# TuringLang/Bijectors.jl

Measured on NVIDIA B200. Metric: samples/sec: with_logabsdet_jacobian through 8-layer Planar flow, D=128, higher is better.
Workload: dtype f32

## Files before the change

### bijectors.jl_b200/csrc/b2b_planar_common.cuh

```cuda
#pragma once
#include <cstring>

#include "b2b_v1_pipeline.cuh"

namespace b2b {

constexpr int HP_MAX_L = 8;
constexpr int HP_MAX_D = 128;

template <int D, int L>
__device__ __forceinline__ void planar_derive_smem(const B2BChainParams& P, int nreal, float* params, int warp, int lane,
                                                   int nw) {
  for (int l = warp; l < L; l += nw) {
    float* w_out = params + l * D;
    float* u_out = params + L * D + l * D;
    if (l >= nreal) {
      for (int i = lane; i < D; i += 32) w_out[i] = u_out[i] = 0.f;
      if (lane == 0) params[2 * L * D + l] = params[2 * L * D + L + l] = 0.f;
      continue;
    }
    const b2b_layer_desc& d = P.layers[l];
    float s = 0.f, q = 0.f;
    for (int i = lane; i < D; i += 32) {
      const float w = d.p0[i], u = d.p1[i];
      s = fmaf(w, u, s);
      q = fmaf(w, w, q);
    }
    s = warp_sum(s);
    q = warp_sum(q);
    const float k = (softplus(-s) - 1.0f) / q;
    for (int i = lane; i < D; i += 32) {
      const float w = d.p0[i];
      w_out[i] = w;
      u_out[i] = fmaf(k, w, d.p1[i]);
    }
    if (lane == 0) {
      params[2 * L * D + l] = softplus(s) - 1.0f;
      params[2 * L * D + L + l] = d.p2[0];
    }
  }
}

static __global__ void __launch_bounds__(HP_MAX_L * 32)
    planar_prep_kernel(const __grid_constant__ B2BChainParams P, int L, int Lp, float* __restrict__ out) {
  const int lane = threadIdx.x & 31, l = threadIdx.x >> 5, D = P.D;
  if (l >= Lp) return;
  auto put = [&](int idx, float v) { out[idx] = v; };
  const int wo = l * D, uo = Lp * D + l * D;
  if (l >= L) {
    for (int i = lane; i < D; i += 32) {
      put(wo + i, 0.f);
      put(uo + i, 0.f);
    }
    if (lane == 0) {
      put(2 * Lp * D + l, 0.f);
      put(2 * Lp * D + Lp + l, 0.f);
    }
    return;
  }
  const b2b_layer_desc& d = P.layers[l];
  float s = 0.f, q = 0.f;
  for (int i = lane; i < D; i += 32) {
    const float w = d.p0[i], u = d.p1[i];
    s = fmaf(w, u, s);
    q = fmaf(w, w, q);
  }
  s = warp_sum(s);
  q = warp_sum(q);
  const float k = (softplus(-s) - 1.0f) / q;
  for (int i = lane; i < D; i += 32) {
    const float w = d.p0[i];
    put(wo + i, w);
    put(uo + i, fmaf(k, w, d.p1[i]));
  }
  if (lane == 0) {
    put(2 * Lp * D + l, softplus(s) - 1.0f);
    put(2 * Lp * D + Lp + l, d.p2[0]);
  }
}

struct HPShape {
  int nw, mode;
};

static HPShape hp_shape(int D, int L) {
  HPShape s;
  s.nw = D == 128 ? 8 : (D == 64 ? 12 : 16);
  s.mode = (2 * D * L * 4 > 4096) ? 2 : 0;
  return s;
}

}
```

### bijectors.jl_b200/csrc/b2b_planar_const.cu

```cuda
#include "b2b_planar_common.cuh"

namespace b2b {

template <int D, int L>
struct PlanarHP {
  float v[2 * L * D + 2 * L];
};

template <int D, int L>
struct ArgSrc {
  static constexpr bool kDerive = false;
  const PlanarHP<D, L>& H;
  int invmask;
  __device__ __forceinline__ float w(int l, int i) const { return H.v[l * D + i]; }
  __device__ __forceinline__ float uh(int l, int i) const { return H.v[L * D + l * D + i]; }
  __device__ __forceinline__ float c(int l) const { return H.v[2 * L * D + l]; }
  __device__ __forceinline__ float b(int l) const { return H.v[2 * L * D + L + l]; }
  __device__ __forceinline__ bool inv(int l) const { return (invmask >> l) & 1; }
  __device__ __forceinline__ float raw(int i) const { return H.v[i]; }
};

template <int D, int L>
struct DevSrc {
  static constexpr bool kDerive = true;
  int invmask, nreal;
  __device__ __forceinline__ bool inv(int l) const { return (invmask >> l) & 1; }
};

template <int D, int L, int MODE, int DIR, bool MVN, class Src>
struct PlanarConstProg {
  using State = V1NoState;
  const Src src;
  const B2BChainParams& P;
  static constexpr bool DERIVE = Src::kDerive;
  static constexpr int NPK = 2 * L * D + 2 * L;
  static constexpr bool STAGED = MODE != 0 || DERIVE;
  static constexpr int MVN_OFF = STAGED ? ((NPK + 3) & ~3) : 0;
  static constexpr bool TAB = DERIVE && DIR != 0;
  static constexpr int TAB_OFF = MVN_OFF + (MVN ? 2 * D + 4 : 0);
  static constexpr int SMEM_FLOATS = TAB_OFF + (TAB ? L * PT_FLOATS : 0);
  __device__ __forceinline__ void stage(float* params, int warp, int lane, int nw) const {
    if constexpr (DERIVE) {
      if (MVN && warp == nw - 1) stage_layer(P.layers[src.nreal], params + MVN_OFF, D, D, lane);
      planar_derive_smem<D, L>(P, src.nreal, params, warp, lane, nw);
      if constexpr (TAB) {
        __syncthreads();
        for (int idx = warp * 32 + lane; idx < L * PT_N; idx += nw * 32) {
          const int l = idx / PT_N;
          if (DIR == 1 || src.inv(l)) planar_table_piece(params[2 * L * D + l], idx - l * PT_N, params + TAB_OFF + l * PT_FLOATS);
        }
      }
    } else if constexpr (STAGED) {
      for (int i = warp * 32 + lane; i < NPK; i += nw * 32) params[i] = src.raw(i);
    }
  }

  template <bool WS, bool US, bool SS>
  __device__ __forceinline__ void layers(float2 (&x)[1][D / 2], const float* params, float (&lj)[1]) const {
#pragma unroll
    for (int l = 0; l < L; ++l) {
      const float4* w4 = reinterpret_cast<const float4*>(params + l * D);
      const float4* u4 = reinterpret_cast<const float4*>(params + L * D + l * D);
      float2 acc[4];
#pragma unroll
      for (int i = 0; i < 4; ++i) acc[i] = make_float2(0.f, 0.f);
#pragma unroll
      for (int i = 0; i < D / 4; ++i) {
        float4 w;
        if constexpr (WS) w = w4[i];
        else w = make_float4(src.w(l, 4 * i), src.w(l, 4 * i + 1), src.w(l, 4 * i + 2), src.w(l, 4 * i + 3));
        acc[(i & 1) * 2 + 0] = __ffma2_rn(make_float2(w.x, w.y), x[0][2 * i], acc[(i & 1) * 2 + 0]);
        acc[(i & 1) * 2 + 1] = __ffma2_rn(make_float2(w.z, w.w), x[0][2 * i + 1], acc[(i & 1) * 2 + 1]);
      }
      const float2 s = __fadd2_rn(__fadd2_rn(acc[0], acc[1]), __fadd2_rn(acc[2], acc[3]));
      const float wz = s.x + s.y;
      float cc_, bb;
      if constexpr (SS) {
        cc_ = params[2 * L * D + l];
        bb = params[2 * L * D + L + l];
      } else {
        cc_ = src.c(l);
        bb = src.b(l);
      }
      float t, s2;
      if (DIR == 0 || (DIR == 2 && !src.inv(l))) {
        tanh_sech2(wz + bb, t, s2);
        lj[0] += log1pf(cc_ * s2);
      } else {
        if constexpr (TAB) find_alpha_tab(wz, cc_, bb, params + TAB_OFF + l * PT_FLOATS, t, s2);
        else find_alpha_ts(wz, cc_, bb, t, s2);
        lj[0] -= log1pf(cc_ * s2);
        t = -t;
      }
      const float2 t2 = make_float2(t, t);
#pragma unroll
      for (int i = 0; i < D / 4; ++i) {
        float4 u;
        if constexpr (US) u = u4[i];
        else u = make_float4(src.uh(l, 4 * i), src.uh(l, 4 * i + 1), src.uh(l, 4 * i + 2), src.uh(l, 4 * i + 3));
        x[0][2 * i] = __ffma2_rn(make_float2(u.x, u.y), t2, x[0][2 * i]);
        x[0][2 * i + 1] = __ffma2_rn(make_float2(u.z, u.w), t2, x[0][2 * i + 1]);
      }
    }
  }

  __device__ __forceinline__ void apply(float2 (&x)[1][D / 2], const ColCtx<D, 1>& ctx, const float* params,
                                        float (&lj)[1]) const {
    if constexpr (DERIVE) layers<true, true, true>(x, params, lj);
    else layers<MODE == 2, MODE == 1, false>(x, params, lj);
    if (MVN) mvnormal_apply<D, 1, 1>(x, ctx, params + MVN_OFF, lj);
  }
};

template <int D, int L, int NW, int MODE, int DIR>
__global__ void __launch_bounds__(NW * 32, 1)
    planar_arg_kernel(const __grid_constant__ B2BChainParams P, const __grid_constant__ V1Extra E,
                      const __grid_constant__ CUtensorMap map_x, const __grid_constant__ CUtensorMap map_y,
                      const __grid_constant__ PlanarHP<D, L> H, const int invmask) {
  const PlanarConstProg<D, L, MODE, DIR, false, ArgSrc<D, L>> prog{{H, invmask}, P};
  v1_run<D, 1, 1, NW>(P, E, map_x, map_y, prog);
}

template <int D, int L, int NW, int DIR, bool MVN>
__global__ void __launch_bounds__(NW * 32, 1)
    planar_dev_kernel(const __grid_constant__ B2BChainParams P, const __grid_constant__ V1Extra E,
                      const __grid_constant__ CUtensorMap map_x, const __grid_constant__ CUtensorMap map_y,
                      const int invmask, const int nreal) {
  const PlanarConstProg<D, L, 0, DIR, MVN, DevSrc<D, L>> prog{{invmask, nreal}, P};
  v1_run<D, 1, 1, NW>(P, E, map_x, map_y, prog);
}

template <int D, int L, int NW, int MODE, int DIR>
static int launch_arg(const B2BChainParams& q, const V1Geom& g, const CUtensorMap& mx, const CUtensorMap& my,
                      const float* packed, int invmask, cudaStream_t stream) {
  static PlanarHP<D, L> H;
  static std::mutex mu;
  std::lock_guard<std::mutex> lock(mu);
  memcpy(H.v, packed, sizeof(H.v));
  auto kernel = planar_arg_kernel<D, L, NW, MODE, DIR>;
  cudaError_t e = cudaFuncSetAttribute(kernel, cudaFuncAttributeMaxDynamicSharedMemorySize, (int)g.smem);
  if (e != cudaSuccess) return (int)e;
  kernel<<<g.grid, NW * 32, g.smem, stream>>>(q, g.extra, mx, my, H, invmask);
  return (int)cudaGetLastError();
}

template <int D, int L, int NW, int DIR, bool MVN = false>
static int launch_dev(const B2BChainParams& q, const V1Geom& g, const CUtensorMap& mx, const CUtensorMap& my,
                      int nreal, int invmask, cudaStream_t stream) {
  auto kernel = planar_dev_kernel<D, L, NW, DIR, MVN>;
  cudaError_t e = cudaFuncSetAttribute(kernel, cudaFuncAttributeMaxDynamicSharedMemorySize, (int)g.smem);
  if (e != cudaSuccess) return (int)e;
  kernel<<<g.grid, NW * 32, g.smem, stream>>>(q, g.extra, mx, my, invmask, nreal);
  return (int)cudaGetLastError();
}

template <int D, int NW, int LL, int MM>
static int dispatch_arg_dir(const B2BChainParams& q, const V1Geom& g, const CUtensorMap& mx, const CUtensorMap& my,
                            const float* packed, int invmask, cudaStream_t stream) {
  const int all = (1 << LL) - 1;
  const int dir = (invmask & all) == 0 ? 0 : ((invmask & all) == all ? 1 : 2);
  if (dir == 0) return launch_arg<D, LL, NW, MM, 0>(q, g, mx, my, packed, invmask, stream);
  if (dir == 1) return launch_arg<D, LL, NW, MM, 1>(q, g, mx, my, packed, invmask, stream);
  return launch_arg<D, LL, NW, MM, 2>(q, g, mx, my, packed, invmask, stream);
}

template <int D, int NW>
static int dispatch_arg(int L, int mode, const B2BChainParams& q, const V1Geom& g, const CUtensorMap& mx,
                        const CUtensorMap& my, const float* packed, int invmask, cudaStream_t stream) {
  if (L == 1 && mode == 0) return dispatch_arg_dir<D, NW, 1, 0>(q, g, mx, my, packed, invmask, stream);
  if (L == 2 && mode == 0) return dispatch_arg_dir<D, NW, 2, 0>(q, g, mx, my, packed, invmask, stream);
  if (L == 4 && mode == 0) return dispatch_arg_dir<D, NW, 4, 0>(q, g, mx, my, packed, invmask, stream);
  if constexpr (2 * D * 8 * 4 > 4096) {
    if (L == 8 && mode == 2) return dispatch_arg_dir<D, NW, 8, 2>(q, g, mx, my, packed, invmask, stream);
  } else {
    if (L == 8 && mode == 0) return dispatch_arg_dir<D, NW, 8, 0>(q, g, mx, my, packed, invmask, stream);
  }
  return B2B_EUNSUPPORTED;
}

template <int D, int NW, int LL>
static int dispatch_dev_dir(const B2BChainParams& q, const V1Geom& g, const CUtensorMap& mx, const CUtensorMap& my,
                            int nreal, int invmask, bool mvn, cudaStream_t stream) {
  const int all = (1 << LL) - 1;
  const int dir = (invmask & all) == 0 ? 0 : ((invmask & all) == all ? 1 : 2);
  if (mvn) {
    if (dir == 1) return launch_dev<D, LL, NW, 1, true>(q, g, mx, my, nreal, invmask, stream);
    return B2B_EUNSUPPORTED;
  }
  if (dir == 0) return launch_dev<D, LL, NW, 0>(q, g, mx, my, nreal, invmask, stream);
  if (dir == 1) return launch_dev<D, LL, NW, 1>(q, g, mx, my, nreal, invmask, stream);
  return launch_dev<D, LL, NW, 2>(q, g, mx, my, nreal, invmask, stream);
}

template <int D, int NW>
static int dispatch_dev(int L, const B2BChainParams& q, const V1Geom& g, const CUtensorMap& mx, const CUtensorMap& my,
                        int nreal, int invmask, bool mvn, cudaStream_t stream) {
  switch (L) {
    case 1: return dispatch_dev_dir<D, NW, 1>(q, g, mx, my, nreal, invmask, mvn, stream);
    case 2: return dispatch_dev_dir<D, NW, 2>(q, g, mx, my, nreal, invmask, mvn, stream);
    case 3: return dispatch_dev_dir<D, NW, 3>(q, g, mx, my, nreal, invmask, mvn, stream);
    case 4: return dispatch_dev_dir<D, NW, 4>(q, g, mx, my, nreal, invmask, mvn, stream);
    case 5: return dispatch_dev_dir<D, NW, 5>(q, g, mx, my, nreal, invmask, mvn, stream);
    case 6: return dispatch_dev_dir<D, NW, 6>(q, g, mx, my, nreal, invmask, mvn, stream);
    case 7: return dispatch_dev_dir<D, NW, 7>(q, g, mx, my, nreal, invmask, mvn, stream);
    case 8: return dispatch_dev_dir<D, NW, 8>(q, g, mx, my, nreal, invmask, mvn, stream);
    default: return B2B_EUNSUPPORTED;
  }
}

static int launch_planar_unrolled(const B2BChainParams& p, int L, const float* packed, int nreal, int invmask, bool mvn,
                                  cudaStream_t stream) {
  B2BChainParams q = p;
  q.scratch_off = -1;
  if (!(q.D == 32 || q.D == 64 || q.D == 128)) return B2B_EUNSUPPORTED;
  if (v1_check_io(q) != 0) return B2B_EUNSUPPORTED;
  const HPShape sh = hp_shape(q.D, L);
  V1Geom g;
  const bool staged = sh.mode != 0 || !packed;
  const size_t pf = (staged ? (size_t)((2 * L * q.D + 2 * L + 3) & ~3) : 0) + (mvn ? 2 * q.D + 4 : 0) +
                    ((!packed && invmask != 0) ? (size_t)L * PT_FLOATS : 0);
  const int rc = v1_geometry(q.D, q.N, sh.nw, 32, pf, g);
  if (rc != 0) return rc;
  CUtensorMap mx, my;
  if (!make_maps(q, g.cols, &mx, &my, &g.extra.tma3d)) return B2B_EUNSUPPORTED;
  if (packed) {
    if (q.D == 128) return dispatch_arg<128, 8>(L, sh.mode, q, g, mx, my, packed, invmask, stream);
    if (q.D == 64) return dispatch_arg<64, 12>(L, sh.mode, q, g, mx, my, packed, invmask, stream);
    return dispatch_arg<32, 16>(L, sh.mode, q, g, mx, my, packed, invmask, stream);
  }
  if (q.D == 128) return dispatch_dev<128, 8>(L, q, g, mx, my, nreal, invmask, mvn, stream);
  if (q.D == 64) return dispatch_dev<64, 12>(L, q, g, mx, my, nreal, invmask, mvn, stream);
  return dispatch_dev<32, 16>(L, q, g, mx, my, nreal, invmask, mvn, stream);
}

}

int b2b_planar_const_grid_size(const B2BChainParams& p) {
  using namespace b2b;
  if (!(p.D == 32 || p.D == 64 || p.D == 128)) return 0;
  V1Geom g;
  const HPShape sh = hp_shape(p.D, 8);
  if (v1_geometry(p.D, p.N, sh.nw, 32, 0, g) != 0) return 0;
  return g.grid;
}

int b2b_launch_planar_hostparams(const B2BChainParams& p, int L, const float* packed, int invmask,
                                 cudaStream_t stream) {
  return b2b::launch_planar_unrolled(p, L, packed, L, invmask, false, stream);
}

int b2b_planar_const_layers(const B2BChainParams& p) {
  using namespace b2b;
  if (!(p.D == 32 || p.D == 64 || p.D == 128) || p.L < 1) return 0;
  const bool mvn = p.layers[p.L - 1].kind == B2B_MVNORMAL_DIAG;
  const int n = p.L - (mvn ? 1 : 0);
  if (n < 1 || n > HP_MAX_L) return 0;
  for (int l = 0; l < n; ++l) {
    if (p.layers[l].kind != B2B_PLANAR) return 0;
    if (mvn && !p.layers[l].inverse) return 0;
  }
  if (v1_check_io(p) != 0) return 0;
  return n;
}

int b2b_launch_planar_chain_const(const B2BChainParams& p, cudaStream_t stream) {
  using namespace b2b;
  const int n = b2b_planar_const_layers(p);
  if (n == 0) return B2B_EUNSUPPORTED;
  int invmask = 0;
  for (int l = 0; l < n; ++l)
    if (p.layers[l].inverse) invmask |= 1 << l;
  return launch_planar_unrolled(p, n, nullptr, n, invmask, p.L > n, stream);
}
```

### bijectors.jl_b200/csrc/b2b_v1_pipeline.cuh

```cuda
#pragma once
#include <cuda.h>
#include <cuda_runtime.h>

#include <cstdlib>
#include <mutex>

#include "b2b_device.cuh"

namespace b2b {

__device__ __forceinline__ uint32_t smem_u32(const void* p) {
  return static_cast<uint32_t>(__cvta_generic_to_shared(p));
}
__device__ __forceinline__ void mbar_init(uint32_t bar, uint32_t count) {
  asm volatile("mbarrier.init.shared::cta.b64 [%0], %1;" ::"r"(bar), "r"(count));
}
__device__ __forceinline__ void mbar_expect_tx(uint32_t bar, uint32_t bytes) {
  asm volatile("mbarrier.arrive.expect_tx.shared::cta.b64 _, [%0], %1;" ::"r"(bar), "r"(bytes) : "memory");
}
__device__ __forceinline__ void mbar_wait(uint32_t bar, uint32_t parity) {
  asm volatile(
      "{\n"
      ".reg .pred P1;\n"
      "B2B_WAIT:\n"
      "mbarrier.try_wait.parity.shared::cta.b64 P1, [%0], %1;\n"
      "@P1 bra B2B_DONE;\n"
      "bra B2B_WAIT;\n"
      "B2B_DONE:\n"
      "}\n" ::"r"(bar),
      "r"(parity)
      : "memory");
}
__device__ __forceinline__ void tma_load_2d(uint32_t dst, const CUtensorMap* map, int c0, int c1, uint32_t bar) {
  asm volatile(
      "cp.async.bulk.tensor.2d.shared::cluster.global.mbarrier::complete_tx::bytes [%0], [%1, {%2, %3}], [%4];" ::"r"(dst),
      "l"(reinterpret_cast<uint64_t>(map)), "r"(c0), "r"(c1), "r"(bar)
      : "memory");
}
__device__ __forceinline__ void tma_store_2d(const CUtensorMap* map, int c0, int c1, uint32_t src) {
  asm volatile("cp.async.bulk.tensor.2d.global.shared::cta.bulk_group [%0, {%1, %2}], [%3];" ::"l"(
                   reinterpret_cast<uint64_t>(map)),
               "r"(c0), "r"(c1), "r"(src)
               : "memory");
}
__device__ __forceinline__ void tma_load_3d(uint32_t dst, const CUtensorMap* map, int c0, int c1, int c2, uint32_t bar) {
  asm volatile(
      "cp.async.bulk.tensor.3d.shared::cluster.global.mbarrier::complete_tx::bytes [%0], [%1, {%2, %3, %4}], [%5];" ::"r"(dst),
      "l"(reinterpret_cast<uint64_t>(map)), "r"(c0), "r"(c1), "r"(c2), "r"(bar)
      : "memory");
}
__device__ __forceinline__ void tma_store_3d(const CUtensorMap* map, int c0, int c1, int c2, uint32_t src) {
  asm volatile("cp.async.bulk.tensor.3d.global.shared::cta.bulk_group [%0, {%1, %2, %3}], [%4];" ::"l"(
                   reinterpret_cast<uint64_t>(map)),
               "r"(c0), "r"(c1), "r"(c2), "r"(src)
               : "memory");
}
__device__ __forceinline__ void mbar_arrive(uint32_t bar) {
  asm volatile("mbarrier.arrive.shared::cta.b64 _, [%0];" ::"r"(bar) : "memory");
}
__device__ __forceinline__ void bulk_load_1d(uint32_t dst, const void* src, uint32_t bytes, uint32_t bar) {
  asm volatile("cp.async.bulk.shared::cluster.global.mbarrier::complete_tx::bytes [%0], [%1], %2, [%3];" ::"r"(dst),
               "l"(reinterpret_cast<uint64_t>(src)), "r"(bytes), "r"(bar)
               : "memory");
}
__device__ __forceinline__ void tma_commit() { asm volatile("cp.async.bulk.commit_group;" ::: "memory"); }
__device__ __forceinline__ void tma_wait_read0() { asm volatile("cp.async.bulk.wait_group.read 0;" ::: "memory"); }
__device__ __forceinline__ void tma_wait_all0() { asm volatile("cp.async.bulk.wait_group 0;" ::: "memory"); }
__device__ __forceinline__ void fence_proxy_async() { asm volatile("fence.proxy.async.shared::cta;" ::: "memory"); }
__device__ __forceinline__ void fence_mbar_init() { asm volatile("fence.mbarrier_init.release.cluster;" ::: "memory"); }
__device__ __forceinline__ void flag_store_release(int* p, int v) {
  asm volatile("st.release.cta.shared::cta.s32 [%0], %1;" ::"r"(smem_u32(p)), "r"(v) : "memory");
}
__device__ __forceinline__ int flag_load_acquire(const int* p) {
  int v;
  asm volatile("ld.acquire.cta.shared::cta.s32 %0, [%1];" : "=r"(v) : "r"(smem_u32(p)) : "memory");
  return v;
}

struct V1Extra {
  int n_in;
  int param_off;
  int bar_off;
  int nwarps;
  int tma3d;
  long long tiles;
};

template <int D, int TPC>
struct ColCtx {
  static constexpr int EPT = D / TPC;
  static constexpr int NQT = EPT / 32;
  int h, rot;
  __device__ __forceinline__ int prm(int ql, int r) const { return (h * NQT + ql) * 8 + (r ^ rot); }
  __device__ __forceinline__ int row(int ql, int r, int e) const { return prm(ql, r) * 4 + e; }
};

template <int TPC>
__device__ __forceinline__ float part_sum(float v) {
#pragma unroll
  for (int o = 1; o < TPC; o <<= 1) v += __shfl_xor_sync(0xffffffffu, v, o);
  return v;
}

#define B2B_FOR_SLOTS                        \
  _Pragma("unroll") for (int ql = 0; ql < C::NQT; ++ql) _Pragma("unroll") for (int r = 0; r < 8; ++r)
#define B2B_FOR_COLS _Pragma("unroll") for (int cc = 0; cc < CPT; ++cc)

template <int D, int TPC, int CPT>
__device__ __forceinline__ void radial_apply(float2 (&x)[CPT][D / TPC / 2], const ColCtx<D, TPC>& c, const float* sp,
                                             bool inverse, float (&lj)[CPT]) {
  using C = ColCtx<D, TPC>;
  const float4* z4 = reinterpret_cast<const float4*>(sp);
  const float alpha = sp[D], bhat = sp[D + 1], apb = sp[D + 2];
  const float2 m1 = make_float2(-1.f, -1.f);
  float2 acc[CPT][4];
  B2B_FOR_COLS {
#pragma unroll
    for (int i = 0; i < 4; ++i) acc[cc][i] = make_float2(0.f, 0.f);
  }
  B2B_FOR_SLOTS {
    const float4 z0 = z4[c.prm(ql, r)];
    const int i = (ql * 8 + r) * 2;
    B2B_FOR_COLS {
      const float2 d0 = __ffma2_rn(make_float2(z0.x, z0.y), m1, x[cc][i]);
      const float2 d1 = __ffma2_rn(make_float2(z0.z, z0.w), m1, x[cc][i + 1]);
      acc[cc][(r & 1) * 2 + 0] = __ffma2_rn(d0, d0, acc[cc][(r & 1) * 2 + 0]);
      acc[cc][(r & 1) * 2 + 1] = __ffma2_rn(d1, d1, acc[cc][(r & 1) * 2 + 1]);
    }
  }
  float2 g2[CPT];
  B2B_FOR_COLS {
    const float2 s = __fadd2_rn(__fadd2_rn(acc[cc][0], acc[cc][1]), __fadd2_rn(acc[cc][2], acc[cc][3]));
    const float nrm = sqrtf(part_sum<TPC>(s.x + s.y));
    float r_ = nrm;
    if (inverse) {
      const float a = apb - nrm;
      const float sq = sqrtf(fmaf(a, a, 4.0f * alpha * nrm));
      r_ = a > 0.f ? (2.0f * alpha * nrm) / (sq + a) : 0.5f * (sq - a);
    }
    const float hh = 1.0f / (alpha + r_);
    const float bh = bhat * hh;
    const float ljf = (float)(D - 1) * log1pf(bh) + log1pf(bh * alpha * hh);
    float g;
    if (!inverse) {
      g = bh;
      lj[cc] += ljf;
    } else {
      g = -bhat / (apb + r_);
      lj[cc] -= ljf;
    }
    g2[cc] = make_float2(g, g);
  }
  B2B_FOR_SLOTS {
    const float4 z0 = z4[c.prm(ql, r)];
    const int i = (ql * 8 + r) * 2;
    B2B_FOR_COLS {
      const float2 d0 = __ffma2_rn(make_float2(z0.x, z0.y), m1, x[cc][i]);
      const float2 d1 = __ffma2_rn(make_float2(z0.z, z0.w), m1, x[cc][i + 1]);
      x[cc][i] = __ffma2_rn(g2[cc], d0, x[cc][i]);
      x[cc][i + 1] = __ffma2_rn(g2[cc], d1, x[cc][i + 1]);
    }
  }
}

template <int D, int TPC, int CPT>
__device__ __forceinline__ void mvnormal_apply(const float2 (&x)[CPT][D / TPC / 2], const ColCtx<D, TPC>& c,
                                               const float* sp, float (&lj)[CPT]) {
  using C = ColCtx<D, TPC>;
  const float4* mu4 = reinterpret_cast<const float4*>(sp);
  const float4* is4 = reinterpret_cast<const float4*>(sp + D);
  const float2 m1 = make_float2(-1.f, -1.f);
  float2 acc[CPT][2];
  B2B_FOR_COLS acc[cc][0] = acc[cc][1] = make_float2(0.f, 0.f);
  B2B_FOR_SLOTS {
    const float4 mu = mu4[c.prm(ql, r)], is = is4[c.prm(ql, r)];
    const int i = (ql * 8 + r) * 2;
    B2B_FOR_COLS {
      const float2 z0 = __fmul2_rn(__ffma2_rn(make_float2(mu.x, mu.y), m1, x[cc][i]), make_float2(is.x, is.y));
      const float2 z1 = __fmul2_rn(__ffma2_rn(make_float2(mu.z, mu.w), m1, x[cc][i + 1]), make_float2(is.z, is.w));
      acc[cc][0] = __ffma2_rn(z0, z0, acc[cc][0]);
      acc[cc][1] = __ffma2_rn(z1, z1, acc[cc][1]);
    }
  }
  B2B_FOR_COLS {
    const float2 s = __fadd2_rn(acc[cc][0], acc[cc][1]);
    lj[cc] += sp[2 * D] - 0.5f * part_sum<TPC>(s.x + s.y);
  }
}

struct V1Gen {
  unsigned long long seed, offset;
  long long col0;
  const float* mu;
  const float* sigma;
};

__device__ __forceinline__ void philox4x32_10(uint32_t c0, uint32_t c1, uint32_t c2, uint32_t c3, uint32_t k0, uint32_t k1,
                                              uint32_t (&out)[4]) {
#pragma unroll
  for (int r = 0; r < 10; ++r) {
    const uint32_t hi0 = __umulhi(0xD2511F53u, c0), lo0 = 0xD2511F53u * c0;
    const uint32_t hi1 = __umulhi(0xCD9E8D57u, c2), lo1 = 0xCD9E8D57u * c2;
    c0 = hi1 ^ c1 ^ k0;
    c1 = lo1;
    c2 = hi0 ^ c3 ^ k1;
    c3 = lo0;
    k0 += 0x9E3779B9u;
    k1 += 0xBB67AE85u;
  }
  out[0] = c0;
  out[1] = c1;
  out[2] = c2;
  out[3] = c3;
}

__device__ __forceinline__ void box_muller(uint32_t a, uint32_t b, float& z0, float& z1) {
  const float u1 = fmaf(__uint2float_rn(a), 2.3283064365386963e-10f, 1.1641532182693481e-10f);
  const float u2 = fmaf(__uint2float_rn(b), 2.3283064365386963e-10f, 1.1641532182693481e-10f);
  const float r = sqrtf(-1.3862943611198906f * __log2f(u1));
  const float ang = 6.283185307179586f * u2 - 3.141592653589793f;
  z0 = -r * __cosf(ang);
  z1 = -r * __sinf(ang);
}

__device__ __forceinline__ float4 philox_normal4(const V1Gen& g, long long n, int k) {
  uint32_t o[4];
  philox4x32_10((uint32_t)n, (uint32_t)((unsigned long long)n >> 32), (uint32_t)k, (uint32_t)g.offset, (uint32_t)g.seed,
                (uint32_t)(g.seed >> 32), o);
  float4 z;
  box_muller(o[0], o[1], z.x, z.y);
  box_muller(o[2], o[3], z.z, z.w);
  return z;
}

struct V1NoState {};

template <int D, int TPC, int CPT, int NW, class Prog, int NIN = 1, bool GEN = false>
__device__ __forceinline__ void v1_run(const B2BChainParams& P, const V1Extra& E, const CUtensorMap& map_x,
                                       const CUtensorMap& map_y, const Prog& prog,
                                       const CUtensorMap* map_x2 = nullptr, const V1Gen* gen = nullptr) {
  using C = ColCtx<D, TPC>;
  constexpr int NQ = D / 32;
  constexpr int LPC = 32 / TPC;
  constexpr int COLS = LPC * CPT;
  constexpr int BOX_BYTES = COLS * 128;
  constexpr int TILE_BYTES = NQ * BOX_BYTES;
  constexpr int SLOT_BYTES = NIN * TILE_BYTES;
  extern __shared__ unsigned char smem_dyn[];
  unsigned char* smem_raw = smem_dyn + ((1024u - (smem_u32(smem_dyn) & 1023u)) & 1023u);
  unsigned char* in_base = smem_raw;
  unsigned char* out_base = smem_raw + (size_t)E.n_in * SLOT_BYTES;
  float* params = reinterpret_cast<float*>(smem_raw + E.param_off);
  uint64_t* bars = reinterpret_cast<uint64_t*>(smem_raw + E.bar_off);
  int* armed = reinterpret_cast<int*>(bars + 8);

  const int lane = threadIdx.x & 31, warp = __shfl_sync(0xffffffffu, (int)(threadIdx.x >> 5), 0);
  auto load_tile = [&](uint32_t dst, int col0, uint32_t bar) {
    if (E.tma3d) {
      tma_load_3d(dst, &map_x, 0, col0, 0, bar);
      if (NIN == 2) tma_load_3d(dst + TILE_BYTES, map_x2, 0, col0, 0, bar);
    } else {
#pragma unroll
      for (int q = 0; q < NQ; ++q) tma_load_2d(dst + q * BOX_BYTES, &map_x, q * 32, col0, bar);
      if (NIN == 2) {
#pragma unroll
        for (int q = 0; q < NQ; ++q) tma_load_2d(dst + TILE_BYTES + q * BOX_BYTES, map_x2, q * 32, col0, bar);
      }
    }
  };
  const long long my_tiles = (E.tiles - blockIdx.x + gridDim.x - 1) / gridDim.x;
  if (threadIdx.x == 0 && !GEN) {
    for (int i = 0; i < E.n_in; ++i) mbar_init(smem_u32(&bars[i]), 1);
    fence_mbar_init();
    for (int j = 0; j < E.n_in && j < my_tiles; ++j) {
      const uint32_t bar = smem_u32(&bars[j]);
      mbar_expect_tx(bar, SLOT_BYTES);
      const long long tile = blockIdx.x + (long long)j * gridDim.x;
      load_tile(smem_u32(in_base + (size_t)j * SLOT_BYTES), (int)(tile * COLS), bar);
      flag_store_release(&armed[j], j);
    }
  }
  prog.stage(params, warp, lane, NW);
  __syncthreads();

  C ctx;
  const int t = lane / TPC;
  ctx.h = lane % TPC;
  ctx.rot = ctx.h * (8 / TPC);
  unsigned char* my_out = out_base + (size_t)warp * TILE_BYTES;
  const int sw = (((t & 7) ^ ctx.rot) & 7) * 16;
  const int line = t * 128 + ctx.h * C::NQT * BOX_BYTES;
  double dsum = 0.0;
  bool store_pending = false;

  for (long long j = warp; j < my_tiles; j += NW) {
    const int buf = (int)(j % E.n_in);
    const uint32_t parity = (uint32_t)((j / E.n_in) & 1);
    const long long tile = blockIdx.x + j * gridDim.x;
    const long long col = tile * COLS + t;
    if constexpr (!GEN) {
      while (flag_load_acquire(&armed[buf]) != (int)j) __nanosleep(20);
      mbar_wait(smem_u32(&bars[buf]), parity);
    }

    float2 x[CPT][C::EPT / 2];
    auto load_fragment = [&](const unsigned char* src) {
      B2B_FOR_COLS {
        B2B_FOR_SLOTS {
          const float4 v =
              *reinterpret_cast<const float4*>(src + cc * (LPC * 128) + ql * BOX_BYTES + ((r * 16) ^ sw));
          x[cc][(ql * 8 + r) * 2] = make_float2(v.x, v.y);
          x[cc][(ql * 8 + r) * 2 + 1] = make_float2(v.z, v.w);
        }
      }
    };
    if constexpr (GEN) {
      B2B_FOR_COLS {
        const long long n = gen->col0 + col + cc * LPC;
        B2B_FOR_SLOTS {
          const int row0 = ctx.row(ql, r, 0);
          float4 z = philox_normal4(*gen, n, row0 >> 2);
          if (gen->sigma) {
            const float4 sg = __ldg(reinterpret_cast<const float4*>(gen->sigma + row0));
            z = make_float4(z.x * sg.x, z.y * sg.y, z.z * sg.z, z.w * sg.w);
          }
          if (gen->mu) {
            const float4 m = __ldg(reinterpret_cast<const float4*>(gen->mu + row0));
            z = make_float4(z.x + m.x, z.y + m.y, z.z + m.z, z.w + m.w);
          }
          x[cc][(ql * 8 + r) * 2] = make_float2(z.x, z.y);
          x[cc][(ql * 8 + r) * 2 + 1] = make_float2(z.z, z.w);
        }
      }
    } else {
      load_fragment(in_base + (size_t)buf * SLOT_BYTES + line);
    }
    typename Prog::State st;
    if constexpr (NIN == 2) {
      prog.phase1(x, ctx, params, st);
      load_fragment(in_base + (size_t)buf * SLOT_BYTES + TILE_BYTES + line);
    }
    if constexpr (!GEN) fence_proxy_async();
    __syncwarp();
    if (!GEN && lane == 0 && j + E.n_in < my_tiles) {
      const uint32_t bar = smem_u32(&bars[buf]);
      mbar_expect_tx(bar, SLOT_BYTES);
      const long long nt = blockIdx.x + (j + E.n_in) * gridDim.x;
      load_tile(smem_u32(in_base + (size_t)buf * SLOT_BYTES), (int)(nt * COLS), bar);
      flag_store_release(&armed[buf], (int)(j + E.n_in));
    }

    float lj[CPT];
    B2B_FOR_COLS {
      const long long cl = col + cc * LPC;
      lj[cc] = (P.accumulate && P.logjac && cl < P.N) ? P.logjac[cl] : 0.0f;
    }
    if constexpr (NIN == 2) prog.apply(x, ctx, params, lj, st, col);
    else prog.apply(x, ctx, params, lj);

    if (P.y) {
      if (store_pending) {
        if (lane == 0) tma_wait_read0();
        __syncwarp();
      }
      unsigned char* dst = my_out + line;
      B2B_FOR_COLS {
        B2B_FOR_SLOTS {
          const float2 a = x[cc][(ql * 8 + r) * 2], b = x[cc][(ql * 8 + r) * 2 + 1];
          *reinterpret_cast<float4*>(dst + cc * (LPC * 128) + ql * BOX_BYTES + ((r * 16) ^ sw)) =
              make_float4(a.x, a.y, b.x, b.y);
        }
      }
      fence_proxy_async();
      __syncwarp();
      if (lane == 0) {
        if (E.tma3d) {
          tma_store_3d(&map_y, 0, (int)(tile * COLS), 0, smem_u32(my_out));
        } else {
#pragma unroll
          for (int q = 0; q < NQ; ++q)
            tma_store_2d(&map_y, q * 32, (int)(tile * COLS), smem_u32(my_out + q * BOX_BYTES));
        }
        tma_commit();
      }
      store_pending = true;
    }
    if (ctx.h == 0) {
      B2B_FOR_COLS {
        const long long cl = col + cc * LPC;
        if (cl < P.N) {
          if (P.logjac && !(P.accumulate & 2)) P.logjac[cl] = lj[cc];
          dsum += (double)lj[cc];
        }
      }
    }
  }
  if (lane == 0 && store_pending) tma_wait_all0();

  if (P.partials) {
    __shared__ double red[32];
#pragma unroll
    for (int o = 16; o > 0; o >>= 1) dsum += __shfl_xor_sync(0xffffffffu, dsum, o);
    if (lane == 0) red[warp] = dsum;
    __syncthreads();
    if (threadIdx.x == 0) {
      double tt = 0.0;
      for (int w = 0; w < NW; ++w) tt += red[w];
      P.partials[blockIdx.x] = tt;
    }
  }
}

typedef CUresult (*encode_tiled_fn)(CUtensorMap*, CUtensorMapDataType, cuuint32_t, void*, const cuuint64_t*,
                                    const cuuint64_t*, const cuuint32_t*, const cuuint32_t*, CUtensorMapInterleave,
                                    CUtensorMapSwizzle, CUtensorMapL2promotion, CUtensorMapFloatOOBfill);

static inline encode_tiled_fn get_encode() {
  static encode_tiled_fn fn = nullptr;
  static std::once_flag once;
  std::call_once(once, [] {
    void* p = nullptr;
    cudaDriverEntryPointQueryResult q;
    if (cudaGetDriverEntryPoint("cuTensorMapEncodeTiled", &p, cudaEnableDefault, &q) == cudaSuccess &&
        q == cudaDriverEntryPointSuccess)
      fn = reinterpret_cast<encode_tiled_fn>(p);
  });
  return fn;
}

static inline bool make_map(CUtensorMap* m, const float* base, int D, long long N, long long ld, int cols, bool three_d) {
  encode_tiled_fn enc = get_encode();
  if (!enc) return false;
  const cuuint32_t estr[3] = {1, 1, 1};
  if (three_d) {
    const cuuint64_t dims[3] = {32, (cuuint64_t)N, (cuuint64_t)(D / 32)};
    const cuuint64_t strides[2] = {(cuuint64_t)ld * sizeof(float), 128};
    const cuuint32_t box[3] = {32, (cuuint32_t)cols, (cuuint32_t)(D / 32)};
    return enc(m, CU_TENSOR_MAP_DATA_TYPE_FLOAT32, 3, const_cast<float*>(base), dims, strides, box, estr,
               CU_TENSOR_MAP_INTERLEAVE_NONE, CU_TENSOR_MAP_SWIZZLE_128B, CU_TENSOR_MAP_L2_PROMOTION_L2_128B,
               CU_TENSOR_MAP_FLOAT_OOB_FILL_NONE) == CUDA_SUCCESS;
  }
  const cuuint64_t dims[2] = {(cuuint64_t)D, (cuuint64_t)N};
  const cuuint64_t strides[1] = {(cuuint64_t)ld * sizeof(float)};
  const cuuint32_t box[2] = {32, (cuuint32_t)cols};
  return enc(m, CU_TENSOR_MAP_DATA_TYPE_FLOAT32, 2, const_cast<float*>(base), dims, strides, box, estr,
             CU_TENSOR_MAP_INTERLEAVE_NONE, CU_TENSOR_MAP_SWIZZLE_128B, CU_TENSOR_MAP_L2_PROMOTION_L2_128B,
             CU_TENSOR_MAP_FLOAT_OOB_FILL_NONE) == CUDA_SUCCESS;
}

static inline bool make_maps(const B2BChainParams& q, int cols, CUtensorMap* mx, CUtensorMap* my, int* tma3d) {
  static const int force2d = getenv("B2B_V1_TMA") && atoi(getenv("B2B_V1_TMA")) == 2;
  for (int three_d = force2d ? 0 : 1; three_d >= 0; --three_d) {
    if (three_d && q.D == 32) continue;
    bool ok = make_map(mx, q.x, q.D, q.N, q.ldx, cols, three_d != 0);
    if (ok && q.y) ok = make_map(my, q.y, q.D, q.N, q.ldy, cols, three_d != 0);
    if (ok) {
      if (!q.y) *my = *mx;
      *tma3d = three_d;
      return true;
    }
  }
  return false;
}

struct V1Geom {
  int nw, grid, cols;
  size_t smem;
  V1Extra extra;
};

static inline int v1_check_io(const B2BChainParams& p) {
  if (p.N >= (1ll << 31) - 64) return B2B_EUNSUPPORTED;
  if ((p.ldx % 4) || (reinterpret_cast<uintptr_t>(p.x) & 15)) return B2B_EUNSUPPORTED;
  if (p.y && ((p.ldy % 4) || (reinterpret_cast<uintptr_t>(p.y) & 15))) return B2B_EUNSUPPORTED;
  return 0;
}

static inline int v1_geometry(int D, long long N, int nw, int cols, size_t param_floats, V1Geom& g,
                              int in_tiles = 1) {
  const int tile_bytes = D * 4 * cols;
  const size_t param_bytes = param_floats * sizeof(float);
  const size_t budget = 225 * 1024;
  const size_t fixed = (size_t)nw * tile_bytes + ((param_bytes + 15) & ~(size_t)15) + 16 * sizeof(uint64_t) + 1024;
  const size_t slot_bytes = (size_t)in_tiles * tile_bytes;
  if (fixed + 2 * slot_bytes > budget) return B2B_EUNSUPPORTED;
  int n_in = (int)((budget - fixed) / slot_bytes);
  if (n_in > 8) n_in = 8;
  g.nw = nw;
  g.cols = cols;
  g.extra.n_in = n_in;
  g.extra.nwarps = nw;
  g.extra.tma3d = 0;
  g.extra.param_off = n_in * (int)slot_bytes + nw * tile_bytes;
  g.extra.bar_off = g.extra.param_off + (int)((param_bytes + 15) & ~(size_t)15);
  g.extra.tiles = (N + cols - 1) / cols;
  g.smem = (size_t)g.extra.bar_off + 16 * sizeof(uint64_t) + 1024;
  int dev = 0, sms = 0;
  cudaGetDevice(&dev);
  cudaDeviceGetAttribute(&sms, cudaDevAttrMultiProcessorCount, dev);
  long long grid = sms;
  const long long want = (g.extra.tiles + nw - 1) / nw;
  if (grid > want) grid = want;
  if (grid < 1) grid = 1;
  g.grid = (int)grid;
  return 0;
}

}
```

Measured before the change: 5.543 billion.

## Add forward planar tile program with coupling matrix and in-place TMA output

For all-forward planar chains, all L projections w_l·x are computed up front from the input. Later layers' pre-activations are then recovered through a precomputed L×L coupling matrix of w_l·û_k dot products, so the serial dependency on the evolving state is removed. Each tile's columns are split across TPC lanes with shuffle reductions, and the output is written back into the input slot in place. That frees the per-warp output buffer and allows up to 16 pipeline stages. The cost is extra parameter derivation per block, a changed barrier layout, and more register pressure from the L×CPT accumulators.

Result: no change. 5.496 billion, median of 6 (-0.8%).

```diff
diff --git a/bijectors.jl_b200/csrc/b2b_planar_common.cuh b/bijectors.jl_b200/csrc/b2b_planar_common.cuh
--- a/bijectors.jl_b200/csrc/b2b_planar_common.cuh
+++ b/bijectors.jl_b200/csrc/b2b_planar_common.cuh
@@ -38,6 +38,18 @@
       params[2 * L * D + l] = softplus(s) - 1.0f;
       params[2 * L * D + L + l] = d.p2[0];
     }
+  }
+}
+
+template <int D, int L>
+__device__ __forceinline__ void planar_derive_coupling(const float* params, float* m, int warp, int lane, int nw) {
+  for (int idx = warp; idx < L * L; idx += nw) {
+    const int l = idx / L, k = idx - l * L;
+    if (k >= l) continue;
+    float s = 0.f;
+    for (int i = lane; i < D; i += 32) s = fmaf(params[l * D + i], params[L * D + k * D + i], s);
+    s = warp_sum(s);
+    if (lane == 0) m[idx] = s;
   }
 }
 
diff --git a/bijectors.jl_b200/csrc/b2b_planar_const.cu b/bijectors.jl_b200/csrc/b2b_planar_const.cu
--- a/bijectors.jl_b200/csrc/b2b_planar_const.cu
+++ b/bijectors.jl_b200/csrc/b2b_planar_const.cu
@@ -112,6 +112,124 @@
   }
 };
 
+template <int D, int L>
+struct PlanarFwdProg {
+  using State = V1NoState;
+  static constexpr bool kTileIO = true;
+  static constexpr int TPC = D / 32, CPT = 4, OWN = CPT / TPC;
+  static constexpr int M_OFF = (2 * L * D + 2 * L + 3) & ~3;
+  static constexpr int SMEM_FLOATS = M_OFF + L * L;
+  const B2BChainParams& P;
+
+  __device__ __forceinline__ void stage(float* params, int warp, int lane, int nw) const {
+    planar_derive_smem<D, L>(P, L, params, warp, lane, nw);
+    __syncthreads();
+    planar_derive_coupling<D, L>(params, params + M_OFF, warp, lane, nw);
+  }
+
+  __device__ __forceinline__ void tile(const unsigned char* src, unsigned char* dst, const ColCtx<D, TPC>& ctx, int sw,
+                                       const float* params, float (&lj)[OWN]) const {
+    using C = ColCtx<D, TPC>;
+    const float4* w4 = reinterpret_cast<const float4*>(params);
+    const float4* u4 = reinterpret_cast<const float4*>(params + L * D);
+    float2 acc[L][CPT];
+#pragma unroll
+    for (int l = 0; l < L; ++l) {
+      B2B_FOR_COLS acc[l][cc] = make_float2(0.f, 0.f);
+    }
+    B2B_FOR_SLOTS {
+      float4 v[CPT];
+      B2B_FOR_COLS v[cc] = *reinterpret_cast<const float4*>(src + v1_chunk<D, TPC, CPT>(cc, ql, r, sw));
+#pragma unroll
+      for (int l = 0; l < L; ++l) {
+        const float4 w = w4[l * (D / 4) + ctx.prm(ql, r)];
+        B2B_FOR_COLS {
+          acc[l][cc] = __ffma2_rn(make_float2(w.x, w.y), make_float2(v[cc].x, v[cc].y), acc[l][cc]);
+          acc[l][cc] = __ffma2_rn(make_float2(w.z, w.w), make_float2(v[cc].z, v[cc].w), acc[l][cc]);
+        }
+      }
+    }
+    float a[L][CPT];
+#pragma unroll
+    for (int l = 0; l < L; ++l) {
+      B2B_FOR_COLS a[l][cc] = acc[l][cc].x + acc[l][cc].y;
+    }
+#pragma unroll
+    for (int o = TPC / 2, n = CPT / 2; o >= 1; o >>= 1, n >>= 1) {
+      const bool hi = ctx.h & o;
+#pragma unroll
+      for (int k = 0; k < n; ++k) {
+#pragma unroll
+        for (int l = 0; l < L; ++l) {
+          const float send = hi ? a[l][k] : a[l][k + n], keep = hi ? a[l][k + n] : a[l][k];
+          a[l][k] = keep + __shfl_xor_sync(0xffffffffu, send, o);
+        }
+      }
+    }
+    const float* M = params + M_OFF;
+    float t[L][CPT];
+#pragma unroll
+    for (int k = 0; k < OWN; ++k) {
+#pragma unroll
+      for (int l = 0; l < L; ++l) {
+        float al = a[l][k];
+#pragma unroll
+        for (int m = 0; m < l; ++m) al = fmaf(M[l * L + m], t[m][k], al);
+        float s2;
+        tanh_sech2(al + params[2 * L * D + L + l], t[l][k], s2);
+        lj[k] += log1pf(params[2 * L * D + l] * s2);
+      }
+    }
+    if (!dst) return;
+#pragma unroll
+    for (int o = 1, n = OWN; o < TPC; o <<= 1, n <<= 1) {
+      const bool hi = ctx.h & o;
+#pragma unroll
+      for (int k = 0; k < n; ++k) {
+#pragma unroll
+        for (int l = 0; l < L; ++l) {
+          const float mine = t[l][k], other = __shfl_xor_sync(0xffffffffu, mine, o);
+          t[l][k] = hi ? other : mine;
+          t[l][k + n] = hi ? mine : other;
+        }
+      }
+    }
+    float2 t2[L][CPT];
+#pragma unroll
+    for (int l = 0; l < L; ++l) {
+      B2B_FOR_COLS t2[l][cc] = make_float2(t[l][cc], t[l][cc]);
+    }
+    constexpr int NS = C::NQT * 8;
+    float4 v[CPT];
+    B2B_FOR_COLS v[cc] = *reinterpret_cast<const float4*>(src + v1_chunk<D, TPC, CPT>(cc, 0, 0, sw));
+#pragma unroll
+    for (int s = 0; s < NS; ++s) {
+      const int ql = s / 8, r = s % 8;
+      float2 z[CPT][2];
+      B2B_FOR_COLS {
+        z[cc][0] = make_float2(v[cc].x, v[cc].y);
+        z[cc][1] = make_float2(v[cc].z, v[cc].w);
+      }
+      if (s + 1 < NS) {
+        B2B_FOR_COLS v[cc] = *reinterpret_cast<const float4*>(src + v1_chunk<D, TPC, CPT>(cc, (s + 1) / 8, (s + 1) % 8, sw));
+      }
+#pragma unroll
+      for (int l = 0; l < L; ++l) {
+        const float4 u = u4[l * (D / 4) + ctx.prm(ql, r)];
+        B2B_FOR_COLS {
+          z[cc][0] = __ffma2_rn(make_float2(u.x, u.y), t2[l][cc], z[cc][0]);
+          z[cc][1] = __ffma2_rn(make_float2(u.z, u.w), t2[l][cc], z[cc][1]);
+        }
+      }
+      B2B_FOR_COLS *reinterpret_cast<float4*>(dst + v1_chunk<D, TPC, CPT>(cc, ql, r, sw)) =
+          make_float4(z[cc][0].x, z[cc][0].y, z[cc][1].x, z[cc][1].y);
+    }
+  }
+};
+
+constexpr int FWD_NW = 8;
+static inline int fwd_cols(int D) { return 4096 / D; }
+
 template <int D, int L, int NW, int MODE, int DIR>
 __global__ void __launch_bounds__(NW * 32, 1)
     planar_arg_kernel(const __grid_constant__ B2BChainParams P, const __grid_constant__ V1Extra E,
@@ -126,8 +244,13 @@
     planar_dev_kernel(const __grid_constant__ B2BChainParams P, const __grid_constant__ V1Extra E,
                       const __grid_constant__ CUtensorMap map_x, const __grid_constant__ CUtensorMap map_y,
                       const int invmask, const int nreal) {
-  const PlanarConstProg<D, L, 0, DIR, MVN, DevSrc<D, L>> prog{{invmask, nreal}, P};
-  v1_run<D, 1, 1, NW>(P, E, map_x, map_y, prog);
+  if constexpr (DIR == 0 && !MVN) {
+    const PlanarFwdProg<D, L> prog{P};
+    v1_run<D, PlanarFwdProg<D, L>::TPC, PlanarFwdProg<D, L>::CPT, NW>(P, E, map_x, map_y, prog);
+  } else {
+    const PlanarConstProg<D, L, 0, DIR, MVN, DevSrc<D, L>> prog{{invmask, nreal}, P};
+    v1_run<D, 1, 1, NW>(P, E, map_x, map_y, prog);
+  }
 }
 
 template <int D, int L, int NW, int MODE, int DIR>
@@ -187,7 +310,7 @@
     if (dir == 1) return launch_dev<D, LL, NW, 1, true>(q, g, mx, my, nreal, invmask, stream);
     return B2B_EUNSUPPORTED;
   }
-  if (dir == 0) return launch_dev<D, LL, NW, 0>(q, g, mx, my, nreal, invmask, stream);
+  if (dir == 0) return launch_dev<D, LL, FWD_NW, 0>(q, g, mx, my, nreal, invmask, stream);
   if (dir == 1) return launch_dev<D, LL, NW, 1>(q, g, mx, my, nreal, invmask, stream);
   return launch_dev<D, LL, NW, 2>(q, g, mx, my, nreal, invmask, stream);
 }
@@ -217,9 +340,11 @@
   const HPShape sh = hp_shape(q.D, L);
   V1Geom g;
   const bool staged = sh.mode != 0 || !packed;
-  const size_t pf = (staged ? (size_t)((2 * L * q.D + 2 * L + 3) & ~3) : 0) + (mvn ? 2 * q.D + 4 : 0) +
+  const bool fwd = !packed && invmask == 0 && !mvn;
+  const size_t pf = (staged ? (size_t)((2 * L * q.D + 2 * L + 3) & ~3) : 0) + (fwd ? L * L : 0) +
+                    (mvn ? 2 * q.D + 4 : 0) +
                     ((!packed && invmask != 0) ? (size_t)L * PT_FLOATS : 0);
-  const int rc = v1_geometry(q.D, q.N, sh.nw, 32, pf, g);
+  const int rc = v1_geometry(q.D, q.N, fwd ? FWD_NW : sh.nw, fwd ? fwd_cols(q.D) : 32, pf, g, 1, fwd);
   if (rc != 0) return rc;
   CUtensorMap mx, my;
   if (!make_maps(q, g.cols, &mx, &my, &g.extra.tma3d)) return B2B_EUNSUPPORTED;
@@ -238,9 +363,12 @@
 int b2b_planar_const_grid_size(const B2BChainParams& p) {
   using namespace b2b;
   if (!(p.D == 32 || p.D == 64 || p.D == 128)) return 0;
+  const int n = b2b_planar_const_layers(p);
+  bool fwd = n > 0 && n == p.L;
+  for (int l = 0; l < n; ++l) fwd = fwd && !p.layers[l].inverse;
   V1Geom g;
   const HPShape sh = hp_shape(p.D, 8);
-  if (v1_geometry(p.D, p.N, sh.nw, 32, 0, g) != 0) return 0;
+  if (v1_geometry(p.D, p.N, fwd ? FWD_NW : sh.nw, fwd ? fwd_cols(p.D) : 32, 0, g, 1, fwd) != 0) return 0;
   return g.grid;
 }
 
diff --git a/bijectors.jl_b200/csrc/b2b_v1_pipeline.cuh b/bijectors.jl_b200/csrc/b2b_v1_pipeline.cuh
--- a/bijectors.jl_b200/csrc/b2b_v1_pipeline.cuh
+++ b/bijectors.jl_b200/csrc/b2b_v1_pipeline.cuh
@@ -4,6 +4,7 @@
 
 #include <cstdlib>
 #include <mutex>
+#include <type_traits>
 
 #include "b2b_device.cuh"
 
@@ -235,11 +236,24 @@
 
 struct V1NoState {};
 
+template <class Prog, class = void>
+struct V1TileIO : std::false_type {};
+template <class Prog>
+struct V1TileIO<Prog, std::void_t<decltype(Prog::kTileIO)>> : std::bool_constant<Prog::kTileIO> {};
+
+template <int D, int TPC, int CPT>
+__device__ __forceinline__ int v1_chunk(int cc, int ql, int r, int sw) {
+  return cc * (32 / TPC * 128) + ql * (32 / TPC * CPT * 128) + ((r * 16) ^ sw);
+}
+
 template <int D, int TPC, int CPT, int NW, class Prog, int NIN = 1, bool GEN = false>
 __device__ __forceinline__ void v1_run(const B2BChainParams& P, const V1Extra& E, const CUtensorMap& map_x,
                                        const CUtensorMap& map_y, const Prog& prog,
                                        const CUtensorMap* map_x2 = nullptr, const V1Gen* gen = nullptr) {
   using C = ColCtx<D, TPC>;
+  constexpr bool TILE = V1TileIO<Prog>::value;
+  static_assert(!TILE || (NIN == 1 && !GEN && CPT % TPC == 0), "tile programs: one input tensor, CPT a multiple of TPC");
+  constexpr int NLJ = TILE ? CPT / TPC : CPT;
   constexpr int NQ = D / 32;
   constexpr int LPC = 32 / TPC;
   constexpr int COLS = LPC * CPT;
@@ -252,7 +266,7 @@
   unsigned char* out_base = smem_raw + (size_t)E.n_in * SLOT_BYTES;
   float* params = reinterpret_cast<float*>(smem_raw + E.param_off);
   uint64_t* bars = reinterpret_cast<uint64_t*>(smem_raw + E.bar_off);
-  int* armed = reinterpret_cast<int*>(bars + 8);
+  int* armed = reinterpret_cast<int*>(bars + E.n_in);
 
   const int lane = threadIdx.x & 31, warp = __shfl_sync(0xffffffffu, (int)(threadIdx.x >> 5), 0);
   auto load_tile = [&](uint32_t dst, int col0, uint32_t bar) {
@@ -303,94 +317,116 @@
       mbar_wait(smem_u32(&bars[buf]), parity);
     }
 
-    float2 x[CPT][C::EPT / 2];
-    auto load_fragment = [&](const unsigned char* src) {
-      B2B_FOR_COLS {
-        B2B_FOR_SLOTS {
-          const float4 v =
-              *reinterpret_cast<const float4*>(src + cc * (LPC * 128) + ql * BOX_BYTES + ((r * 16) ^ sw));
-          x[cc][(ql * 8 + r) * 2] = make_float2(v.x, v.y);
-          x[cc][(ql * 8 + r) * 2 + 1] = make_float2(v.z, v.w);
+    auto rearm = [&] {
+      if (!GEN && lane == 0 && j + E.n_in < my_tiles) {
+        const uint32_t bar = smem_u32(&bars[buf]);
+        mbar_expect_tx(bar, SLOT_BYTES);
+        const long long nt = blockIdx.x + (j + E.n_in) * gridDim.x;
+        load_tile(smem_u32(in_base + (size_t)buf * SLOT_BYTES), (int)(nt * COLS), bar);
+        flag_store_release(&armed[buf], (int)(j + E.n_in));
+      }
+    };
+    float2 x[TILE ? 1 : CPT][TILE ? 1 : C::EPT / 2];
+    typename Prog::State st;
+    if constexpr (!TILE) {
+      auto load_fragment = [&](const unsigned char* src) {
+        B2B_FOR_COLS {
+          B2B_FOR_SLOTS {
+            const float4 v = *reinterpret_cast<const float4*>(src + v1_chunk<D, TPC, CPT>(cc, ql, r, sw));
+            x[cc][(ql * 8 + r) * 2] = make_float2(v.x, v.y);
+            x[cc][(ql * 8 + r) * 2 + 1] = make_float2(v.z, v.w);
+          }
         }
-      }
-    };
-    if constexpr (GEN) {
-      B2B_FOR_COLS {
-        const long long n = gen->col0 + col + cc * LPC;
-        B2B_FOR_SLOTS {
-          const int row0 = ctx.row(ql, r, 0);
-          float4 z = philox_normal4(*gen, n, row0 >> 2);
-          if (gen->sigma) {
-            const float4 sg = __ldg(reinterpret_cast<const float4*>(gen->sigma + row0));
-            z = make_float4(z.x * sg.x, z.y * sg.y, z.z * sg.z, z.w * sg.w);
+      };
+      if constexpr (GEN) {
+        B2B_FOR_COLS {
+          const long long n = gen->col0 + col + cc * LPC;
+          B2B_FOR_SLOTS {
+            const int row0 = ctx.row(ql, r, 0);
+            float4 z = philox_normal4(*gen, n, row0 >> 2);
+            if (gen->sigma) {
+              const float4 sg = __ldg(reinterpret_cast<const float4*>(gen->sigma + row0));
+              z = make_float4(z.x * sg.x, z.y * sg.y, z.z * sg.z, z.w * sg.w);
+            }
+            if (gen->mu) {
+              const float4 m = __ldg(reinterpret_cast<const float4*>(gen->mu + row0));
+              z = make_float4(z.x + m.x, z.y + m.y, z.z + m.z, z.w + m.w);
+            }
+            x[cc][(ql * 8 + r) * 2] = make_float2(z.x, z.y);
+            x[cc][(ql * 8 + r) * 2 + 1] = make_float2(z.z, z.w);
           }
-          if (gen->mu) {
-            const float4 m = __ldg(reinterpret_cast<const float4*>(gen->mu + row0));
-            z = make_float4(z.x + m.x, z.y + m.y, z.z + m.z, z.w + m.w);
-          }
-          x[cc][(ql * 8 + r) * 2] = make_float2(z.x, z.y);
-          x[cc][(ql * 8 + r) * 2 + 1] = make_float2(z.z, z.w);
         }
-      }
-    } else {
-      load_fragment(in_base + (size_t)buf * SLOT_BYTES + line);
-    }
-    typename Prog::State st;
-    if constexpr (NIN == 2) {
-      prog.phase1(x, ctx, params, st);
-      load_fragment(in_base + (size_t)buf * SLOT_BYTES + TILE_BYTES + line);
-    }
-    if constexpr (!GEN) fence_proxy_async();
-    __syncwarp();
-    if (!GEN && lane == 0 && j + E.n_in < my_tiles) {
-      const uint32_t bar = smem_u32(&bars[buf]);
-      mbar_expect_tx(bar, SLOT_BYTES);
-      const long long nt = blockIdx.x + (j + E.n_in) * gridDim.x;
-      load_tile(smem_u32(in_base + (size_t)buf * SLOT_BYTES), (int)(nt * COLS), bar);
-      flag_store_release(&armed[buf], (int)(j + E.n_in));
-    }
-
-    float lj[CPT];
-    B2B_FOR_COLS {
-      const long long cl = col + cc * LPC;
-      lj[cc] = (P.accumulate && P.logjac && cl < P.N) ? P.logjac[cl] : 0.0f;
-    }
-    if constexpr (NIN == 2) prog.apply(x, ctx, params, lj, st, col);
-    else prog.apply(x, ctx, params, lj);
-
-    if (P.y) {
-      if (store_pending) {
-        if (lane == 0) tma_wait_read0();
-        __syncwarp();
-      }
-      unsigned char* dst = my_out + line;
-      B2B_FOR_COLS {
-        B2B_FOR_SLOTS {
-          const float2 a = x[cc][(ql * 8 + r) * 2], b = x[cc][(ql * 8 + r) * 2 + 1];
-          *reinterpret_cast<float4*>(dst + cc * (LPC * 128) + ql * BOX_BYTES + ((r * 16) ^ sw)) =
-              make_float4(a.x, a.y, b.x, b.y);
-        }
-      }
+      } else {
+        load_fragment(in_base + (size_t)buf * SLOT_BYTES + line);
+      }
+      if constexpr (NIN == 2) {
+        prog.phase1(x, ctx, params, st);
+        load_fragment(in_base + (size_t)buf * SLOT_BYTES + TILE_BYTES + line);
+      }
+      if constexpr (!GEN) fence_proxy_async();
+      __syncwarp();
+      rearm();
+    }
+
+    const int lj0 = TILE ? ctx.h * NLJ : 0;
+    float lj[NLJ];
+#pragma unroll
+    for (int k = 0; k < NLJ; ++k) {
+      const long long cl = col + (lj0 + k) * LPC;
+      lj[k] = (P.accumulate && P.logjac && cl < P.N) ? P.logjac[cl] : 0.0f;
+    }
+    unsigned char* const slot = in_base + (size_t)buf * SLOT_BYTES;
+    unsigned char* const ytile = TILE ? slot : my_out;
+    if constexpr (TILE) {
+      prog.tile(slot + line, P.y ? slot + line : nullptr, ctx, sw, params, lj);
       fence_proxy_async();
       __syncwarp();
+    } else if constexpr (NIN == 2) {
+      prog.apply(x, ctx, params, lj, st, col);
+    } else {
+      prog.apply(x, ctx, params, lj);
+    }
+
+    if (P.y) {
+      if constexpr (!TILE) {
+        if (store_pending) {
+          if (lane == 0) tma_wait_read0();
+          __syncwarp();
+        }
+        unsigned char* dst = my_out + line;
+        B2B_FOR_COLS {
+          B2B_FOR_SLOTS {
+            const float2 a = x[cc][(ql * 8 + r) * 2], b = x[cc][(ql * 8 + r) * 2 + 1];
+            *reinterpret_cast<float4*>(dst + v1_chunk<D, TPC, CPT>(cc, ql, r, sw)) = make_float4(a.x, a.y, b.x, b.y);
+          }
+        }
+        fence_proxy_async();
+        __syncwarp();
+      }
       if (lane == 0) {
         if (E.tma3d) {
-          tma_store_3d(&map_y, 0, (int)(tile * COLS), 0, smem_u32(my_out));
+          tma_store_3d(&map_y, 0, (int)(tile * COLS), 0, smem_u32(ytile));
         } else {
 #pragma unroll
           for (int q = 0; q < NQ; ++q)
-            tma_store_2d(&map_y, q * 32, (int)(tile * COLS), smem_u32(my_out + q * BOX_BYTES));
+            tma_store_2d(&map_y, q * 32, (int)(tile * COLS), smem_u32(ytile + q * BOX_BYTES));
         }
         tma_commit();
       }
       store_pending = true;
     }
-    if (ctx.h == 0) {
-      B2B_FOR_COLS {
-        const long long cl = col + cc * LPC;
+    if constexpr (TILE) {
+      if (P.y && lane == 0) tma_wait_read0();
+      rearm();
+      __syncwarp();
+    }
+    if (TILE || ctx.h == 0) {
+#pragma unroll
+      for (int k = 0; k < NLJ; ++k) {
+        const long long cl = col + (lj0 + k) * LPC;
         if (cl < P.N) {
-          if (P.logjac && !(P.accumulate & 2)) P.logjac[cl] = lj[cc];
-          dsum += (double)lj[cc];
+          if (P.logjac && !(P.accumulate & 2)) P.logjac[cl] = lj[k];
+          dsum += (double)lj[k];
         }
       }
     }
@@ -477,24 +513,26 @@
 }
 
 static inline int v1_geometry(int D, long long N, int nw, int cols, size_t param_floats, V1Geom& g,
-                              int in_tiles = 1) {
+                              int in_tiles = 1, bool in_place = false) {
   const int tile_bytes = D * 4 * cols;
   const size_t param_bytes = param_floats * sizeof(float);
+  const size_t bar_bytes = (in_place ? 32 : 16) * sizeof(uint64_t);
   const size_t budget = 225 * 1024;
-  const size_t fixed = (size_t)nw * tile_bytes + ((param_bytes + 15) & ~(size_t)15) + 16 * sizeof(uint64_t) + 1024;
+  const size_t fixed =
+      (in_place ? 0 : (size_t)nw * tile_bytes) + ((param_bytes + 15) & ~(size_t)15) + bar_bytes + 1024;
   const size_t slot_bytes = (size_t)in_tiles * tile_bytes;
   if (fixed + 2 * slot_bytes > budget) return B2B_EUNSUPPORTED;
   int n_in = (int)((budget - fixed) / slot_bytes);
-  if (n_in > 8) n_in = 8;
+  if (n_in > (in_place ? 16 : 8)) n_in = in_place ? 16 : 8;
   g.nw = nw;
   g.cols = cols;
   g.extra.n_in = n_in;
   g.extra.nwarps = nw;
   g.extra.tma3d = 0;
-  g.extra.param_off = n_in * (int)slot_bytes + nw * tile_bytes;
+  g.extra.param_off = n_in * (int)slot_bytes + (in_place ? 0 : nw * tile_bytes);
   g.extra.bar_off = g.extra.param_off + (int)((param_bytes + 15) & ~(size_t)15);
   g.extra.tiles = (N + cols - 1) / cols;
-  g.smem = (size_t)g.extra.bar_off + 16 * sizeof(uint64_t) + 1024;
+  g.smem = (size_t)g.extra.bar_off + bar_bytes + 1024;
   int dev = 0, sms = 0;
   cudaGetDevice(&dev);
   cudaDeviceGetAttribute(&sms, cudaDevAttrMultiProcessorCount, dev);
```
